# simeoncarstens/binf

Measured on AMD Instinct MI355X. Metric: chain*leapfrog-steps/sec, 1024-d Gaussian, higher is better.
Workload: dtype f64

## Files before the change

### binf_amd/csrc/hmc_gauss_kernel.hpp

```cpp
#pragma once
#include "gauss_common.hpp"
#include "xoshiro.hpp"

namespace binf {

enum { GAUSS_RNG_HBM = 0, GAUSS_RNG_FUSED = 1, GAUSS_RNG_DUMP = 2 };

constexpr int gauss_wpb(int LW, int RNG) { return (LW == 3 || RNG != GAUSS_RNG_HBM) ? 8 : 4; }

constexpr int GAUSS_STEP_UNROLL = 4;
constexpr int gauss_step_unroll(int TMAX, bool REGULAR, bool UNIT, bool FMA, int LW, int RNG)
{
    if (!REGULAR || LW != 0 || !UNIT) return 1;
    if ((TMAX == 12 && !FMA) || (TMAX == 4 && RNG == GAUSS_RNG_FUSED)) return 1;
    return GAUSS_STEP_UNROLL;
}

constexpr int GAUSS_PRIO_WINDOW = 4;
constexpr bool gauss_wave_priority(int LW, int RNG, int HC)
{
    return LW == 0 && RNG == GAUSS_RNG_HBM && HC == 3;
}

__device__ __forceinline__ void gauss_set_priority(int prio)
{
    switch (prio & 3) {
    case 0: __builtin_amdgcn_s_setprio(0); break;
    case 1: __builtin_amdgcn_s_setprio(1); break;
    case 2: __builtin_amdgcn_s_setprio(2); break;
    default: __builtin_amdgcn_s_setprio(3); break;
    }
}

constexpr int GAUSS_REDO_GS = 2;
template <int TMAX, int GS, bool UNIT, bool FMA, bool WIDE = false>
__device__ inline bool gauss_exact_accept(const GaussNArgs &a, const double *qs, const double (*qs_lds)[64],
                                          int lane, const double *pc, double dt, double hdt, double c_lp,
                                          double u)
{
    LaneSum s0 = {0.0, 0.0}, spb = {0.0, 0.0}, sqa = {0.0, 0.0}, spa = {0.0, 0.0};
    const int e0 = 128 * (lane >> 3) + (lane & 7);
#pragma unroll 1
    for (int g = 0; g < TMAX / GS; ++g) {
        double qq[GS], pp[GS];
#pragma unroll
        for (int i = 0; i < GS; ++i) {
            const int t = g * GS + i;
            if (WIDE) qq[i] = qs_lds ? (&qs_lds[0][0])[e0 + 8 * t] : qs[8 * t];
            else qq[i] = qs_lds ? qs_lds[t][lane] : qs[8 * t];
            pp[i] = pc[8 * t];
        }
#pragma unroll
        for (int i = 0; i < GS; ++i) {
            const int t = g * GS + i;
            const double d = UNIT ? qq[i] : qq[i] - a.x0;
            lane_sum_add<true>(s0, d * d, t, TMAX);
            lane_sum_add<true>(spb, pp[i] * pp[i], t, TMAX);
        }
#pragma unroll
        for (int i = 0; i < GS; ++i)
            pp[i] = kick<FMA>(pp[i], hdt, gauss_grad<UNIT>(qq[i], a.k, a.x0));
#pragma unroll 1
        for (int l = 0; l < a.nsteps - 1; ++l) {
#pragma unroll
            for (int i = 0; i < GS; ++i) {
                qq[i] = drift<FMA>(qq[i], pp[i], dt);
                pp[i] = kick<FMA>(pp[i], dt, gauss_grad<UNIT>(qq[i], a.k, a.x0));
            }
        }
#pragma unroll
        for (int i = 0; i < GS; ++i) {
            const int t = g * GS + i;
            qq[i] = drift<FMA>(qq[i], pp[i], dt);
            pp[i] = kick<FMA>(pp[i], hdt, gauss_grad<UNIT>(qq[i], a.k, a.x0));
            const double d = UNIT ? qq[i] : qq[i] - a.x0;
            lane_sum_add<true>(sqa, d * d, t, TMAX);
            lane_sum_add<true>(spa, pp[i] * pp[i], t, TMAX);
        }
    }
    const double r = chain_sums_shared(sqa.r, spa.r, spb.r, s0.r, true);
    const double Eb = -(c_lp * lane_value_f64<12>(r)) + 0.5 * lane_value_f64<8>(r);
    const double Ea = -(c_lp * lane_value_f64<0>(r)) + 0.5 * lane_value_f64<4>(r);
    return metropolis_accept<true>(u, -(Ea - Eb));
}

constexpr int GAUSS_STREAM_NT_RECORD = 1;
constexpr int GAUSS_STREAM_NT_P0 = 2;
constexpr int GAUSS_STREAM_WIDE = GAUSS_STREAM_NT_RECORD | GAUSS_STREAM_NT_P0;
constexpr int gauss_stream_policy(bool WIDE) { return WIDE ? GAUSS_STREAM_WIDE : 0; }

constexpr bool gauss_fastsum_built(int TMAX, int HC, bool UNIT) { return HC == 3 && (TMAX == 16 || !UNIT); }

typedef double gauss_d2 __attribute__((ext_vector_type(2)));
template <bool NT = false>
__device__ __forceinline__ void gauss_ld2(double &x, double &y, const double *p)
{
    const gauss_d2 v = NT ? __builtin_nontemporal_load(reinterpret_cast<const gauss_d2 *>(p))
                          : *reinterpret_cast<const gauss_d2 *>(p);
    x = v.x;
    y = v.y;
}
template <bool NT = false>
__device__ __forceinline__ void gauss_st2(double *p, double x, double y)
{
    const gauss_d2 v = {x, y};
    if (NT) __builtin_nontemporal_store(v, reinterpret_cast<gauss_d2 *>(p));
    else *reinterpret_cast<gauss_d2 *>(p) = v;
}

template <int TMAX, bool REGULAR, bool UNIT, bool FMA, int LW, int RNG = GAUSS_RNG_HBM, bool UDT = false,
          int HC = -1, bool FASTSUM = false, bool ONESUM = false, bool WIDE = false>
__global__ void __launch_bounds__(64 * gauss_wpb(LW, RNG))
hmc_gauss_persist_kernel(const GaussNArgs a)
{
    static_assert(!WIDE || (ONESUM && TMAX == 16 && HC == 3 && REGULAR && LW == 0),
                  "16-byte ownership: the two-sum kernel of one 1024-element chain per wave");
    static_assert(HC < 0 || (REGULAR && LW == 0), "compile-time tree height: regular one-wave chains only");
    constexpr bool FIXED = HC >= 0;
    constexpr int HF = FIXED ? HC : 0;
    constexpr bool SHARED = HC == 3;
    static_assert(!FASTSUM || (SHARED && RNG == GAUSS_RNG_HBM), "fused sums: the shared-tree kernels, draws from HBM");
    static_assert(!ONESUM || (FASTSUM && UNIT && UDT), "two sums: the unit Gaussian, one step size for the batch");
    constexpr bool EARLY = FIXED && UNIT && !SHARED;
    constexpr int WPB = gauss_wpb(LW, RNG);
    constexpr int WPC = 1 << LW;
    __shared__ double xch[WPB];
    __shared__ double ubc[WPB];
    constexpr int GS = (TMAX % 8 == 0) ? 8 : ((TMAX % 4 == 0) ? 4 : TMAX);
    constexpr int NG = TMAX / GS;
    constexpr int USTEP = gauss_step_unroll(TMAX, REGULAR, UNIT, FMA, LW, RNG);
    constexpr bool PRIO = gauss_wave_priority(LW, RNG, HC);
    constexpr bool NT_REC = (gauss_stream_policy(WIDE) & GAUSS_STREAM_NT_RECORD) != 0;
    constexpr bool NT_P0 = (gauss_stream_policy(WIDE) & GAUSS_STREAM_NT_P0) != 0;
    alignas(WIDE ? 16 : 8) __shared__ double stash[RNG == GAUSS_RNG_DUMP ? 1 : WPB][RNG == GAUSS_RNG_DUMP ? 1 : TMAX][64];
    __shared__ double zx[RNG == GAUSS_RNG_HBM ? 1 : XZIG_C + 1];
    if (RNG != GAUSS_RNG_HBM) {
        xzig_load_table(zx, threadIdx.x, WPB * 64);
        __syncthreads();
    }

    const int lane = threadIdx.x & 63;
    const int wib = threadIdx.x >> 6;
    const int64_t wave = (int64_t)blockIdx.x * WPB + wib;
    const int H = FIXED ? HC : a.H;
    const int lg = (LW > 0) ? 6 : 3 + H;
    const int slot = lane & ((1 << lg) - 1);
    const int j = slot & 7;
    const int wchain = wib & (WPC - 1);
    const int grp = (LW > 0) ? ((wchain << 3) | (lane >> 3)) : (slot >> 3);
    const bool writer = (LW > 0) ? (wchain == 0 && lane == 0) : (slot == 0);

    int off, n, leafdepth, canonical;
    if (REGULAR) {
        n = 8 * TMAX;
        off = grp * n;
        leafdepth = H;
        canonical = 1;
    } else {
        const Leaf L = pairwise_leaf(a.D, H, grp);
        off = L.off;
        n = L.len;
        leafdepth = L.depth;
        canonical = L.canonical;
    }
    const int T = (n >= 8) ? (n >> 3) : 0;
    const int rem = (n >= 8) ? (n & 7) : n;

    const int64_t raw = (LW > 0) ? (int64_t)blockIdx.x * (WPB / WPC) + (wib >> LW)
                                 : (wave << (6 - lg)) + (lane >> lg);
    const bool cvalid = raw < a.C;
    const int64_t chain = cvalid ? raw : a.C - 1;
    const int64_t CD = a.C * (int64_t)a.D;
    const int64_t base_np = chain * (int64_t)a.D + off + j;
    constexpr int WR0 = TMAX / 4;
    const int64_t base = WIDE ? chain * (int64_t)a.D + 2 * lane + 128 * WR0 : base_np;

    double dt = (UDT || !a.dt_chain) ? a.timestep : a.dt_chain[chain];
    double uu = 0.0;
    if (RNG == GAUSS_RNG_HBM) uu = a.u[chain];
    Xo128 gen = {0u, 0u, 0u, 0u};
    uint64_t gen_stream = 0;
    if (RNG != GAUSS_RNG_HBM) {
        const int cgrp = grp & ~((1 << (H - leafdepth)) - 1);
        gen_stream = (uint64_t)(chain + a.chain_offset) * (uint64_t)(8 << H) + (uint64_t)(cgrp * 8 + j);
    }
    __builtin_amdgcn_sched_barrier(0);

    double q[TMAX], pa[GS], pb[GS];
    if constexpr (WIDE) {
#pragma unroll
        for (int r = 0; r < GS / 2; ++r) gauss_ld2(q[2 * r], q[2 * r + 1], a.q0 + base + 128 * (r - WR0));
#pragma unroll
        for (int r = 0; r < GS / 2; ++r) gauss_ld2<NT_P0>(pa[2 * r], pa[2 * r + 1], a.p0 + base + 128 * (r - WR0));
#pragma unroll
        for (int r = GS / 2; r < TMAX / 2; ++r) gauss_ld2(q[2 * r], q[2 * r + 1], a.q0 + base + 128 * (r - WR0));
    } else {
#pragma unroll
        for (int t = 0; t < GS; ++t) {
            const bool m = REGULAR || (8 * t + j < n);
            q[t] = (m && RNG != GAUSS_RNG_DUMP) ? a.q0[base + 8 * t] : 0.0;
        }
        if (RNG == GAUSS_RNG_HBM) {
#pragma unroll
            for (int i = 0; i < GS; ++i) {
                const bool m = REGULAR || (8 * i + j < n);
                pa[i] = m ? a.p0[base + 8 * i] : 0.0;
            }
        }
#pragma unroll
        for (int t = GS; t < TMAX; ++t) {
            const bool m = REGULAR || (8 * t + j < n);
            q[t] = (m && RNG != GAUSS_RNG_DUMP) ? a.q0[base + 8 * t] : 0.0;
        }
    }

    const double c_lp = SHARED ? a.c_lp : -0.5 * a.k;
    LaneSum s0 = {0.0, 0.0};
    double Sq_state = 0.0;
    int64_t nacc = 0;

    const bool stash_lds = !(REGULAR && ((a.samples && a.thin == 1) || a.n == 1));
    double *rec = a.samples;
    const double *prev = a.q0;
    int rec_wait = a.thin;

    for (int s = 0; s < a.n; ++s) {
        if (PRIO) {
            const int left = (a.n - 1 - s) / GAUSS_PRIO_WINDOW;
            gauss_set_priority(left < 3 ? left : 3);
        }
        const double hdt = (UDT && SHARED) ? a.half_timestep : 0.5 * dt;
        if (RNG != GAUSS_RNG_HBM) gen = xo_seed(gen_stream, a.rng_seed, a.rng_offset + (uint64_t)s);
        if (RNG != GAUSS_RNG_DUMP && stash_lds) {
            if constexpr (WIDE) {
#pragma unroll
                for (int r = 0; r < TMAX / 2; ++r)
                    gauss_st2(&stash[wib][0][0] + 128 * r + 2 * lane, q[2 * r], q[2 * r + 1]);
            } else {
#pragma unroll
                for (int t = 0; t < TMAX; ++t) stash[wib][t][lane] = q[t];
            }
        }

        const bool more = s + 1 < a.n;
        const double *pc = a.p0 + (int64_t)s * CD + base;
        const double *pn = more ? pc + CD : pc;
        double un = 0.0;
        if (RNG == GAUSS_RNG_HBM) un = a.u[(int64_t)(more ? s + 1 : s) * a.C + chain];

        LaneSum spb = {0.0, 0.0}, sqa = {0.0, 0.0}, spa = {0.0, 0.0};
        double Spb = 0.0;
#pragma unroll
        for (int g = 0; g < NG; ++g) {
            double(&cur)[GS] = (RNG == GAUSS_RNG_HBM && (g & 1)) ? pb : pa;
            double(&nxt)[GS] = (RNG == GAUSS_RNG_HBM && (g & 1)) ? pa : pb;
            if (RNG != GAUSS_RNG_HBM) {
                unsigned want = 0;
#pragma unroll
                for (int i = 0; i < GS; ++i)
                    if (REGULAR || (8 * (g * GS + i) + j < n)) want |= 1u << i;
                xzig_normals<GS>(cur, want, gen, zx);
                if (RNG == GAUSS_RNG_DUMP) {
                    if (cvalid && canonical) {
                        double *go = a.p_dump + (int64_t)s * CD + base;
#pragma unroll
                        for (int i = 0; i < GS; ++i)
                            if (want & (1u << i)) go[8 * (g * GS + i)] = cur[i];
                    }
                    continue;
                }
            } else if (WIDE) {
                const double *pg = (g + 1 < NG) ? pc + 128 * ((g + 1) * (GS / 2)) : pn;
#pragma unroll
                for (int r = 0; r < GS / 2; ++r) gauss_ld2<NT_P0>(nxt[2 * r], nxt[2 * r + 1], pg + 128 * (r - WR0));
            } else if (g + 1 < NG) {
#pragma unroll
                for (int i = 0; i < GS; ++i) {
                    const int t = (g + 1) * GS + i;
                    const bool m = REGULAR || (8 * t + j < n);
                    nxt[i] = m ? pc[8 * t] : 0.0;
                }
            } else {
#pragma unroll
                for (int i = 0; i < GS; ++i) {
                    const bool m = REGULAR || (8 * i + j < n);
                    nxt[i] = m ? pn[8 * i] : 0.0;
                }
            }
            (void)nxt;
#pragma unroll
            for (int i = 0; i < GS; ++i)
                asm volatile("" : "+v"(cur[i]), "+v"(q[g * GS + i]));
            if (s == 0) {
#pragma unroll
                for (int i = 0; i < GS; ++i) {
                    const int t = g * GS + i;
                    const double d = UNIT ? q[t] : q[t] - a.x0;
                    if (FASTSUM) lane_sum_fused(s0, d, t);
                    else lane_sum_add<REGULAR>(s0, d * d, t, T);
                }
                if (FIXED && !SHARED && g == NG - 1) {
                    double v[1] = {s0.r};
                    chain_sum_finish_fixed<HF, 1>(v, lane);
                    Sq_state = v[0];
                }
            }
#pragma unroll
            for (int i = 0; i < GS; ++i) {
                if (FASTSUM) lane_sum_fused(spb, cur[i], g * GS + i);
                else lane_sum_add<REGULAR>(spb, cur[i] * cur[i], g * GS + i, T);
            }
            __builtin_amdgcn_sched_barrier(0);
            if (EARLY && g == NG - 1) {
                double v[1] = {spb.r};
                chain_sum_finish_fixed<HF, 1>(v, lane);
                Spb = v[0];
            }
#pragma unroll
            for (int i = 0; i < GS; ++i) {
                const int t = g * GS + i;
                cur[i] = kick<FMA>(cur[i], hdt, gauss_grad<UNIT>(q[t], a.k, a.x0));
            }
            if (EARLY && g == NG - 1) asm volatile("" : "+v"(Spb));
            if (USTEP == 1) {
                for (int l = 0; l < a.nsteps - 1; ++l) {
#pragma unroll
                    for (int i = 0; i < GS; ++i) {
                        const int t = g * GS + i;
                        q[t] = drift<FMA>(q[t], cur[i], dt);
                        cur[i] = kick<FMA>(cur[i], dt, gauss_grad<UNIT>(q[t], a.k, a.x0));
                    }
                }
            } else {
                const auto step = [&]() {
#pragma unroll
                    for (int i = 0; i < GS; ++i) {
                        const int t = g * GS + i;
                        q[t] = drift<FMA>(q[t], cur[i], dt);
                        cur[i] = kick<FMA>(cur[i], dt, gauss_grad<UNIT>(q[t], a.k, a.x0));
                    }
                };
                static_assert((USTEP & (USTEP - 1)) == 0, "the remainder below goes by the bits of its count");
                const int nl = a.nsteps > 1 ? a.nsteps - 1 : 0;
#pragma unroll 1
                for (int m = nl / USTEP; m > 0; --m) {
#pragma unroll
                    for (int k = 0; k < USTEP; ++k) step();
                }
#pragma unroll
                for (int b = USTEP >> 1; b > 0; b >>= 1) {
                    if (nl & b) {
#pragma unroll
                        for (int k = 0; k < b; ++k) step();
                    }
                }
            }
#pragma unroll
            for (int i = 0; i < GS; ++i) {
                const int t = g * GS + i;
                q[t] = drift<FMA>(q[t], cur[i], dt);
                if (!ONESUM) cur[i] = kick<FMA>(cur[i], hdt, gauss_grad<UNIT>(q[t], a.k, a.x0));
            }
#pragma unroll
            for (int i = 0; i < GS; ++i) {
                const int t = g * GS + i;
                const double d = UNIT ? q[t] : q[t] - a.x0;
                if (ONESUM) {
                    lane_sum_fused(sqa, d, t);
                } else if (FASTSUM) {
                    lane_sum_fused(sqa, d, t);
                    lane_sum_fused(spa, cur[i], t);
                } else {
                    lane_sum_add<REGULAR>(sqa, d * d, t, T);
                    lane_sum_add<REGULAR>(spa, cur[i] * cur[i], t, T);
                }
            }
            if (ONESUM)
                asm volatile("" : "+v"(sqa.r), "+v"(spb.r));
            else if (EARLY && g == NG - 1)
                asm volatile("" : "+v"(sqa.r), "+v"(spa.r));
            else
                asm volatile("" : "+v"(sqa.r), "+v"(spa.r), "+v"(spb.r));
            __builtin_amdgcn_sched_barrier(0);
        }
        if (RNG != GAUSS_RNG_HBM) {
            const double ud = xo_uniform53(gen);
            if (LW == 0) {
                uu = shfl_f64(ud, lane & ~((1 << lg) - 1));
            } else {
                if (wchain == 0 && lane == 0) ubc[wib] = ud;
                __syncthreads();
                uu = ubc[wib & ~(WPC - 1)];
                __syncthreads();
            }
            if (RNG == GAUSS_RNG_DUMP) {
                if (cvalid && writer) a.u_dump[(int64_t)s * a.C + chain] = uu;
                continue;
            }
        }
        if (RNG == GAUSS_RNG_HBM && (NG & 1)) {
#pragma unroll
            for (int i = 0; i < GS; ++i) pa[i] = pb[i];
        }
        double Sqa, Spa = 0.0;
        if (ONESUM) {
            const double r = chain_sums_shared2(sqa.r, spb.r, s0.r, s == 0);
            Sqa = lane_value_f64<0>(r);
            Spb = lane_value_f64<4>(r);
            if (s == 0) Sq_state = lane_value_f64<8>(r);
        } else if (SHARED) {
            const double r = chain_sums_shared(sqa.r, spa.r, spb.r, s0.r, s == 0);
            Sqa = lane_value_f64<0>(r);
            Spa = lane_value_f64<4>(r);
            Spb = lane_value_f64<8>(r);
            if (s == 0) Sq_state = lane_value_f64<12>(r);
        } else if (FIXED) {
            if (EARLY) {
                double v[2] = {sqa.r, spa.r};
                chain_sum_finish_fixed<HF, 2>(v, lane);
                Sqa = v[0];
                Spa = v[1];
            } else {
                double v[3] = {spb.r, sqa.r, spa.r};
                chain_sum_finish_fixed<HF, 3>(v, lane);
                Spb = v[0];
                Sqa = v[1];
                Spa = v[2];
            }
        } else {
            if (s == 0)
                Sq_state = chain_sum_finish<REGULAR, LW>(s0, T, rem, lane, H, leafdepth, xch, wib);
            Spb = chain_sum_finish<REGULAR, LW>(spb, T, rem, lane, H, leafdepth, xch, wib);
            Sqa = chain_sum_finish<REGULAR, LW>(sqa, T, rem, lane, H, leafdepth, xch, wib);
            Spa = chain_sum_finish<REGULAR, LW>(spa, T, rem, lane, H, leafdepth, xch, wib);
        }
        const double Eb = -(c_lp * Sq_state) + 0.5 * Spb;
        const double Ea = -(c_lp * Sqa) + 0.5 * Spa;

        bool acc;
        if (FASTSUM) {
            const double xt = ONESUM ? -(a.c_dh * (Sqa - Sq_state)) : -(Ea - Eb);
            const double delta = ONESUM ? a.f_dh * ((Eb + Eb) + __builtin_fabs(xt)) : 0x1p-46 * (Eb + Ea);
            const int dec = accept_decide(uu, xt, delta);
            acc = dec == GAUSS_ACCEPT;
            if (__builtin_amdgcn_ballot_w64(dec == GAUSS_UNDECIDED || !(c_lp < 0.0)) != 0) {
                acc = gauss_exact_accept<TMAX, GAUSS_REDO_GS, UNIT, FMA, WIDE>(
                    a, prev + base_np, stash_lds ? stash[wib] : nullptr, lane, pc + (base_np - base), dt, hdt,
                    c_lp, uu);
                __builtin_amdgcn_s_waitcnt(0);
            }
        } else {
            acc = metropolis_accept<SHARED>(uu, -(Ea - Eb));
        }

        if (!UDT && s < a.n_adapt)
            dt = acc ? dt * a.uprate : dt * a.downrate;
        if (cvalid && writer) {
            const int64_t o = (int64_t)s * a.C + chain;
            if (a.accepted) a.accepted[o] = acc ? 1 : 0;
            if (!ONESUM) {
                if (a.e_before) a.e_before[o] = Eb;
                if (a.e_after) a.e_after[o] = Ea;
            }
        }
        if (acc) {
            Sq_state = Sqa;
            nacc += 1;
        } else {
            if (WIDE && stash_lds) {
#pragma unroll
                for (int r = 0; r < TMAX / 2; ++r)
                    gauss_ld2(q[2 * r], q[2 * r + 1], &stash[wib][0][0] + 128 * r + 2 * lane);
            } else if (WIDE) {
#pragma unroll
                for (int r = 0; r < TMAX / 2; ++r) gauss_ld2(q[2 * r], q[2 * r + 1], prev + base + 128 * (r - WR0));
            } else if (stash_lds) {
#pragma unroll
                for (int t = 0; t < TMAX; ++t) q[t] = stash[wib][t][lane];
            } else {
#pragma unroll
                for (int t = 0; t < TMAX; ++t) q[t] = prev[base + 8 * t];
            }
            __builtin_amdgcn_s_waitcnt(0);
        }
        if (a.samples && --rec_wait == 0) {
            rec_wait = a.thin;
            if (cvalid && canonical) {
                double *go = rec + base;
                if constexpr (WIDE) {
#pragma unroll
                    for (int r = 0; r < TMAX / 2; ++r) gauss_st2<NT_REC>(go + 128 * (r - WR0), q[2 * r], q[2 * r + 1]);
                } else {
#pragma unroll
                    for (int t = 0; t < TMAX; ++t)
                        if (REGULAR || (8 * t + j < n)) go[8 * t] = q[t];
                }
            }
            prev = rec;
            rec += CD;
        }
        if (RNG == GAUSS_RNG_HBM) uu = un;
    }
    if (RNG == GAUSS_RNG_DUMP) return;
    if (PRIO) __builtin_amdgcn_s_setprio(0);

    if (cvalid && writer) {
        if (a.n_accepted) a.n_accepted[chain] += nacc;
        if (!UDT && a.n_adapt > 0 && a.dt_chain) a.dt_chain[chain] = dt;
    }
    if (cvalid && canonical) {
        double *go = a.q_out + base;
        if constexpr (WIDE) {
#pragma unroll
            for (int r = 0; r < TMAX / 2; ++r) gauss_st2(go + 128 * (r - WR0), q[2 * r], q[2 * r + 1]);
        } else {
#pragma unroll
            for (int t = 0; t < TMAX; ++t)
                if (REGULAR || (8 * t + j < n)) go[8 * t] = q[t];
        }
    }
}


}
```

### binf_amd/csrc/hmc_gauss_rng.hip

```cpp
#include "hmc_gauss_rng_launch.hpp"

namespace binf {

template <int RNG>
static hipError_t launch_rng(const GaussNArgs &a, const GaussPlan &p, bool unit, bool fma,
                             hipStream_t st)
{
    if (p.LW > 0) return launch_gauss_rng_wide(a, p, RNG, unit, fma, st);
    const dim3 grid((unsigned)((p.blocks + 1) / 2));
    const int t = p.tneed;
    const bool udt = RNG == GAUSS_RNG_FUSED && !a.dt_chain && a.n_adapt == 0;
#define BINF_RNG_CASE(T)                                                            \
    if (p.regular && t == T && udt)                                                 \
        return launch_rng_tr<T, true, RNG, 0, RNG == GAUSS_RNG_FUSED>(a, unit, fma, grid, st); \
    return (p.regular && t == T) ? launch_rng_tr<T, true, RNG>(a, unit, fma, grid, st) \
                                 : launch_rng_tr<T, false, RNG>(a, unit, fma, grid, st)
    if (t <= 1) { BINF_RNG_CASE(1); }
    if (t <= 2) { BINF_RNG_CASE(2); }
    if (t <= 4) { BINF_RNG_CASE(4); }
    if (t <= 8) { BINF_RNG_CASE(8); }
    if (t <= 12) { BINF_RNG_CASE(12); }
    BINF_RNG_CASE(16);
#undef BINF_RNG_CASE
}

static int32_t rng_plan(const char *what, int64_t C, int64_t D, GaussPlan &p)
{
    if (D > 8192)
        return fail(BINF_E_UNSUPPORTED, "%s: D=%lld > 8192 not covered by the persistent kernel",
                    what, (long long)D);
    p = gauss_plan(C, D);
    if (p.H > 6)
        return fail(BINF_E_UNSUPPORTED, "%s: pairwise tree height %d > 6 for D=%lld", what, p.H,
                    (long long)D);
    if (p.blocks > 0x7fffffffLL) return fail(BINF_E_UNSUPPORTED, "%s: too many chains", what);
    return 0;
}

}

using namespace binf;

extern "C" int32_t binf_hmc_sample_n_gauss_rng_f64(
    const double *q0, double *q_out, double *samples, uint8_t *accepted,
    int64_t *n_accepted, double *e_before, double *e_after, double timestep,
    double *dt_chain, int64_t C, int64_t D, int32_t nsteps, int32_t n, int32_t thin,
    double k, double x0, int32_t n_adapt, double uprate, double downrate, int32_t mode,
    uint64_t seed, uint64_t offset, int64_t chain_offset, void *stream)
{
    const char *what = "hmc_sample_n_gauss_rng";
    if (C < 0 || D < 1 || nsteps < 1 || n < 1 || thin < 1 || n_adapt < 0 || chain_offset < 0)
        return fail(BINF_E_ARG, "%s: need C>=0, D>=1, nsteps>=1, n>=1, thin>=1, n_adapt>=0, "
                    "chain_offset>=0", what);
    if (mode != BINF_MODE_EXACT && mode != BINF_MODE_FMA)
        return fail(BINF_E_ARG, "%s: unknown mode %d", what, mode);
    if (C == 0) return 0;
    if (!q0 || !q_out) return fail(BINF_E_ARG, "%s: null buffer", what);
    if (n_adapt > 0 && !dt_chain) return fail(BINF_E_ARG, "%s: adaption needs dt_chain", what);
    const int64_t bytes = C * D * (int64_t)sizeof(double);
    const char *qo = (const char *)q_out, *qi = (const char *)q0;
    if (qo != qi && qo < qi + bytes && qi < qo + bytes)
        return fail(BINF_E_ALIAS, "%s: q_out overlaps q0 (only q_out == q0 is allowed)", what);
    GaussPlan p;
    if (int32_t rc = rng_plan(what, C, D, p)) return rc;
    GaussNArgs a;
    a.q0 = q0; a.p0 = nullptr; a.u = nullptr; a.q_out = q_out; a.samples = samples;
    a.accepted = accepted; a.n_accepted = n_accepted; a.e_before = e_before;
    a.e_after = e_after; a.dt_chain = dt_chain; a.timestep = timestep; a.k = k;
    a.x0 = x0; a.uprate = uprate; a.downrate = downrate; a.C = C;
    a.D = (int32_t)D; a.nsteps = nsteps; a.H = p.H; a.n = n; a.thin = thin;
    a.n_adapt = n_adapt < n ? n_adapt : n;
    a.rng_seed = seed; a.rng_offset = offset; a.chain_offset = chain_offset;
    a.p_dump = nullptr; a.u_dump = nullptr;
    gauss_derived_args(a);
    const hipError_t e = launch_rng<GAUSS_RNG_FUSED>(a, p, k == 1.0 && x0 == 0.0,
                                                    mode == BINF_MODE_FMA, (hipStream_t)stream);
    if (e != hipSuccess) return hip_fail(e, "hmc_gauss_persist_kernel (fused generator) launch");
    return 0;
}

extern "C" int32_t binf_hmc_gauss_rng_draws_f64(double *p0_out, double *u_out, int64_t C,
                                                int64_t D, int32_t n, uint64_t seed,
                                                uint64_t offset, int64_t chain_offset,
                                                void *stream)
{
    const char *what = "hmc_gauss_rng_draws";
    if (C < 0 || D < 1 || n < 1 || chain_offset < 0)
        return fail(BINF_E_ARG, "%s: need C>=0, D>=1, n>=1, chain_offset>=0", what);
    if (C == 0) return 0;
    if (!p0_out || !u_out) return fail(BINF_E_ARG, "%s: null buffer", what);
    GaussPlan p;
    if (int32_t rc = rng_plan(what, C, D, p)) return rc;
    GaussNArgs a = {};
    a.C = C; a.D = (int32_t)D; a.nsteps = 1; a.H = p.H; a.n = n; a.thin = 1;
    a.k = 1.0;
    a.rng_seed = seed; a.rng_offset = offset; a.chain_offset = chain_offset;
    a.p_dump = p0_out; a.u_dump = u_out;
    gauss_derived_args(a);
    const hipError_t e = launch_rng<GAUSS_RNG_DUMP>(a, p, true, false, (hipStream_t)stream);
    if (e != hipSuccess) return hip_fail(e, "hmc_gauss_persist_kernel (draw dump) launch");
    return 0;
}
```

Before: 5.567 billion.

## Route fused-generator chains through fast-sum shared-tree kernels with regenerated momenta

Adds fused-RNG variants of the fast-sum shared-tree persistent kernels, used for regular 1024-d chains with tree height 3 when no energies are recorded. On the rare exact-accept fallback, the initial momenta are drawn again from the generator rather than read from HBM. This also enables wave priority for these kernels. It aims to cut the cost of the energy reductions and accept test in the fused generator path, at the cost of more kernel instantiations and recomputing random draws when the fallback fires.

Result: no change. 5.561 billion (-0.1%).

```diff
diff --git a/binf_amd/csrc/hmc_gauss_kernel.hpp b/binf_amd/csrc/hmc_gauss_kernel.hpp
--- a/binf_amd/csrc/hmc_gauss_kernel.hpp
+++ b/binf_amd/csrc/hmc_gauss_kernel.hpp
@@ -19,7 +19,7 @@
 constexpr int GAUSS_PRIO_WINDOW = 4;
 constexpr bool gauss_wave_priority(int LW, int RNG, int HC)
 {
-    return LW == 0 && RNG == GAUSS_RNG_HBM && HC == 3;
+    return LW == 0 && RNG != GAUSS_RNG_DUMP && HC == 3;
 }
 
 __device__ __forceinline__ void gauss_set_priority(int prio)
@@ -33,22 +33,37 @@
 }
 
 constexpr int GAUSS_REDO_GS = 2;
-template <int TMAX, int GS, bool UNIT, bool FMA, bool WIDE = false>
+template <int TMAX, int GS, bool UNIT, bool FMA, bool WIDE = false, int RNG = GAUSS_RNG_HBM, int GM = GS>
 __device__ inline bool gauss_exact_accept(const GaussNArgs &a, const double *qs, const double (*qs_lds)[64],
                                           int lane, const double *pc, double dt, double hdt, double c_lp,
-                                          double u)
-{
+                                          double u, Xo128 gen = {0u, 0u, 0u, 0u}, const double *zx = nullptr)
+{
+    static_assert(RNG == GAUSS_RNG_HBM || (RNG == GAUSS_RNG_FUSED && GM % GS == 0 && TMAX % GM == 0),
+                  "drawn again: whole sub-groups of the kernel's groups");
+    static_assert(RNG == GAUSS_RNG_HBM || !WIDE, "a lane's stream is named by numpy's ownership");
     LaneSum s0 = {0.0, 0.0}, spb = {0.0, 0.0}, sqa = {0.0, 0.0}, spa = {0.0, 0.0};
     const int e0 = 128 * (lane >> 3) + (lane & 7);
+    constexpr int SUB = RNG == GAUSS_RNG_FUSED ? GM / GS : 1;
+    static_assert((SUB & (SUB - 1)) == 0, "a drawn group is a power-of-two count of sub-groups");
+    double pm[RNG == GAUSS_RNG_FUSED ? GM : 1];
 #pragma unroll 1
     for (int g = 0; g < TMAX / GS; ++g) {
         double qq[GS], pp[GS];
+        if constexpr (RNG == GAUSS_RNG_FUSED) {
+            if ((g & (SUB - 1)) == 0) xzig_normals<GM>(pm, (1u << GM) - 1u, gen, zx);
+#pragma unroll
+            for (int i = 0; i < GS; ++i) pp[i] = pm[i];
+#pragma unroll
+            for (int i = 0; i + GS < GM; ++i) pm[i] = pm[i + GS];
+#pragma unroll
+            for (int i = 0; i < GM; ++i) asm volatile("" : "+v"(pm[i]));
+        }
 #pragma unroll
         for (int i = 0; i < GS; ++i) {
             const int t = g * GS + i;
             if (WIDE) qq[i] = qs_lds ? (&qs_lds[0][0])[e0 + 8 * t] : qs[8 * t];
             else qq[i] = qs_lds ? qs_lds[t][lane] : qs[8 * t];
-            pp[i] = pc[8 * t];
+            if constexpr (RNG != GAUSS_RNG_FUSED) pp[i] = pc[8 * t];
         }
 #pragma unroll
         for (int i = 0; i < GS; ++i) {
@@ -90,6 +105,10 @@
 constexpr int gauss_stream_policy(bool WIDE) { return WIDE ? GAUSS_STREAM_WIDE : 0; }
 
 constexpr bool gauss_fastsum_built(int TMAX, int HC, bool UNIT) { return HC == 3 && (TMAX == 16 || !UNIT); }
+constexpr bool gauss_rng_fastsum_built(int TMAX, bool UNIT, bool ONESUM)
+{
+    return ONESUM ? TMAX == 16 : (gauss_fastsum_built(TMAX, 3, UNIT) && TMAX == 12);
+}
 
 typedef double gauss_d2 __attribute__((ext_vector_type(2)));
 template <bool NT = false>
@@ -119,7 +138,8 @@
     constexpr bool FIXED = HC >= 0;
     constexpr int HF = FIXED ? HC : 0;
     constexpr bool SHARED = HC == 3;
-    static_assert(!FASTSUM || (SHARED && RNG == GAUSS_RNG_HBM), "fused sums: the shared-tree kernels, draws from HBM");
+    static_assert(!FASTSUM || (SHARED && RNG != GAUSS_RNG_DUMP), "fused sums: the shared-tree kernels that integrate");
+    static_assert(!WIDE || RNG == GAUSS_RNG_HBM, "a generated stream is named by numpy's ownership");
     static_assert(!ONESUM || (FASTSUM && UNIT && UDT), "two sums: the unit Gaussian, one step size for the batch");
     constexpr bool EARLY = FIXED && UNIT && !SHARED;
     constexpr int WPB = gauss_wpb(LW, RNG);
@@ -444,9 +464,17 @@
             const int dec = accept_decide(uu, xt, delta);
             acc = dec == GAUSS_ACCEPT;
             if (__builtin_amdgcn_ballot_w64(dec == GAUSS_UNDECIDED || !(c_lp < 0.0)) != 0) {
-                acc = gauss_exact_accept<TMAX, GAUSS_REDO_GS, UNIT, FMA, WIDE>(
-                    a, prev + base_np, stash_lds ? stash[wib] : nullptr, lane, pc + (base_np - base), dt, hdt,
-                    c_lp, uu);
+                if constexpr (FASTSUM && RNG == GAUSS_RNG_FUSED) {
+                    int sr = s;
+                    asm volatile("" : "+s"(sr));
+                    acc = gauss_exact_accept<TMAX, GAUSS_REDO_GS, UNIT, FMA, false, GAUSS_RNG_FUSED, GS>(
+                        a, prev + base_np, stash_lds ? stash[wib] : nullptr, lane, nullptr, dt, hdt, c_lp, uu,
+                        xo_seed(gen_stream, a.rng_seed, a.rng_offset + (uint64_t)sr), zx);
+                } else {
+                    acc = gauss_exact_accept<TMAX, GAUSS_REDO_GS, UNIT, FMA, WIDE>(
+                        a, prev + base_np, stash_lds ? stash[wib] : nullptr, lane, pc + (base_np - base), dt, hdt,
+                        c_lp, uu);
+                }
                 __builtin_amdgcn_s_waitcnt(0);
             }
         } else {
diff --git a/binf_amd/csrc/hmc_gauss_rng.hip b/binf_amd/csrc/hmc_gauss_rng.hip
--- a/binf_amd/csrc/hmc_gauss_rng.hip
+++ b/binf_amd/csrc/hmc_gauss_rng.hip
@@ -1,6 +1,36 @@
 #include "hmc_gauss_rng_launch.hpp"
 
 namespace binf {
+
+template <int TMAX>
+static hipError_t launch_rng_fastsum(const GaussNArgs &a, bool unit, bool fma, bool udt, dim3 grid,
+                                     hipStream_t st, bool &launched)
+{
+    constexpr int R = GAUSS_RNG_FUSED;
+    launched = true;
+    if constexpr (gauss_rng_fastsum_built(TMAX, true, true)) {
+        if (unit && udt && gauss_onesum_domain(a)) {
+            if (fma) hmc_gauss_persist_kernel<TMAX, true, true, true, 0, R, true, 3, true, true><<<grid, 512, 0, st>>>(a);
+            else     hmc_gauss_persist_kernel<TMAX, true, true, false, 0, R, true, 3, true, true><<<grid, 512, 0, st>>>(a);
+            return hipGetLastError();
+        }
+    }
+    static_assert(!gauss_rng_fastsum_built(TMAX, true, false), "no unit FASTSUM kernel without ONESUM is built");
+    if constexpr (gauss_rng_fastsum_built(TMAX, false, false)) {
+        if (!unit) {
+            if (udt) {
+                if (fma) hmc_gauss_persist_kernel<TMAX, true, false, true, 0, R, true, 3, true><<<grid, 512, 0, st>>>(a);
+                else     hmc_gauss_persist_kernel<TMAX, true, false, false, 0, R, true, 3, true><<<grid, 512, 0, st>>>(a);
+            } else {
+                if (fma) hmc_gauss_persist_kernel<TMAX, true, false, true, 0, R, false, 3, true><<<grid, 512, 0, st>>>(a);
+                else     hmc_gauss_persist_kernel<TMAX, true, false, false, 0, R, false, 3, true><<<grid, 512, 0, st>>>(a);
+            }
+            return hipGetLastError();
+        }
+    }
+    launched = false;
+    return hipSuccess;
+}
 
 template <int RNG>
 static hipError_t launch_rng(const GaussNArgs &a, const GaussPlan &p, bool unit, bool fma,
@@ -10,6 +40,15 @@
     const dim3 grid((unsigned)((p.blocks + 1) / 2));
     const int t = p.tneed;
     const bool udt = RNG == GAUSS_RNG_FUSED && !a.dt_chain && a.n_adapt == 0;
+    if constexpr (RNG == GAUSS_RNG_FUSED) {
+        if (p.regular && p.H == 3 && !a.e_before && !a.e_after) {
+            bool launched = false;
+            hipError_t e = hipSuccess;
+            if (t == 12) e = launch_rng_fastsum<12>(a, unit, fma, udt, grid, st, launched);
+            if (t == 16) e = launch_rng_fastsum<16>(a, unit, fma, udt, grid, st, launched);
+            if (launched) return e;
+        }
+    }
 #define BINF_RNG_CASE(T)                                                            \
     if (p.regular && t == T && udt)                                                 \
         return launch_rng_tr<T, true, RNG, 0, RNG == GAUSS_RNG_FUSED>(a, unit, fma, grid, st); \
```
